# xieydd/crane-scheduler

Hardware: AMD Instinct MI355X
Metric: placements/sec (higher is better)
Workload: dtype f64

## Files before the change

crane-scheduler_amd/csrc/engine.hip:

```cpp
#include <hip/hip_runtime.h>

#include <algorithm>
#include <chrono>
#include <cmath>
#include <cstdio>
#include <cstdlib>
#include <cstring>
#include <memory>
#include <mutex>
#include <string>
#include <vector>

#include "../../include/crane_dyn.h"
#include "bindings.hpp"
#include "dyn_types.hpp"
#include "kernels.hpp"

using namespace crane;

namespace {

hipError_t before_free() { return crane::tl_aql ? crane::aql_wait(crane::tl_aql) : hipSuccess; }

template <typename T>
// ... 517 lines not shown
            HIPTRY(h, launch_step_one(s, st));
            h->reset_deferred = h->defer_reset;
            pk = k1.next;
            k1.on = false;
        } else if (pk.on && mine && pk.q == tl_aql) {
            HIPTRY(h, launch_k3s_delta_pods(h->N, h->node_offset, pk.P, pk.keys, pk.stt, pk.g, pk.perm, pk.pnow,
                                            pk.tiles, h->sd->bnode.p, h->N, d, adj.p, *pods, st));
            pk.on = false;
        } else {
            d.trace = h->trace_region(0);
            if ((pods ? pods->ntiles : 0) + (L + 1023) / 1024 > kTraceWgs) d.trace = nullptr;
            HIPTRY(h, launch_hot_count_delta(h->sd->bnode.p, h->N, d, adj.p, st, pods));
        }
        if (pods_done) *pods_done = pods != nullptr && pods->P > 0;
        h->delta_first = true;
        h->delta_chunks = (L + 1023) / 1024;
    }
    h->dl_adj_dirty[ab] = true;
    h->dl_pending = true;
    *done = true;
    return CRANE_OK;
}

static int hot_values_locked(crane_dyn* h, int64_t now_ns, int64_t hv_ts_ns, hipStream_t st,
                             const PodPrep* pods = nullptr, bool* pods_done = nullptr) {
    if (pods_done) *pods_done = false;
    h->delta_first = false;
    h->reset_deferred = false;
    if (h->N < 0) return h->fail(CRANE_E_STATE, "upload nodes before refreshing hot values");
    DevPolicy& dp = h->dp;
    HotCutoffs cut{};
// ... 1550 lines not shown
```

crane-scheduler_amd/csrc/hotcount.hip:

```cpp
#include <hip/hip_runtime.h>

#include <algorithm>

#include "dyn_types.hpp"
#include "kernels.hpp"
#include "pods.hpp"
#include "lds_hash.hpp"
#include "step_node.hpp"

namespace crane {

__device__ __forceinline__ int window_rank(int64_t ts, const HotCutoffs& cut) {
    int j = 0;
#pragma unroll
    for (int w = 0; w < kMaxWin; ++w)
        if (w < cut.n_win) j += ts > cut.sorted[w] ? 1 : 0;
    return j;
}

constexpr int kXChunk = kHxRegion;


template <int BT, bool POS>
__device__ __forceinline__ void k2d_body(const int32_t blk, const int32_t* __restrict__ bnode,
// ... 149 lines not shown
    for (int k = 1; k <= 4; ++k) CRANE_TSTAMP(d.trace, blockIdx.x, k);
}

hipError_t launch_hot_count_delta(const int32_t* bnode, int64_t N, const HotDelta& d, uint32_t* adj, hipStream_t st,
                                  const PodPrep* pods) {
    constexpr int BT = 512;
    if (d.n_rng < 0 || d.n_rng > kMaxWin || d.n_win < 1 || d.n_win > kDeltaMaxWin || N >= (1LL << 27))
        return hipErrorInvalidValue;
    const int64_t L = d.n_rng > 0 ? d.start[d.n_rng] : 0;
    const int64_t nb = (L + kDeltaChunk - 1) / kDeltaChunk;
    PodPrep pp{};
    if (pods && pods->P > 0) pp = *pods;
    const int64_t grid = pp.ntiles + nb;
    if (grid == 0) return hipSuccess;
    if (grid >= (1LL << 31)) return hipErrorInvalidValue;
    size_t lds = sizeof(uint32_t) * 2 * (size_t)kDeltaSlots + sizeof(uint16_t) * kDeltaMaxWin * kDeltaChunk;
    if (pp.ntiles > 0) lds = std::max(lds, kK3pLds);
    return klaunch(pp.ntiles > 0 ? "k2_delta+k3p_pods" : "k2_delta", k2_delta_pods<BT>, dim3((unsigned)grid), dim3(BT),
                   lds, st, bnode, N, d, adj, pp);
}

template <int BT, int REG, bool POS>
__global__ __launch_bounds__(BT) __attribute__((amdgpu_waves_per_eu(BT == 1024 ? 8 : 1)))
void k2l_partition(const int32_t* __restrict__ bnode,
                                                    const int64_t* __restrict__ bts, int64_t B, int64_t N,
                                                    HotCutoffs cut, HotPart g, uint32_t* __restrict__ CO,
                                                    uint32_t* __restrict__ region) {
    constexpr int kPer = REG / BT;
    constexpr int kSlots = 2 * REG;
    extern __shared__ __attribute__((aligned(16))) uint32_t sh[];
    __shared__ uint32_t part[BT];
// ... 230 lines not shown
```

crane-scheduler_amd/csrc/kernels.hpp:

```cpp
#pragma once
#include <hip/hip_ext.h>
#include <hip/hip_runtime.h>
#include <stdint.h>

#include "aql.hpp"
#include "dyn_types.hpp"

namespace crane {

enum { kShape4x6 = 0, kShape8x8 = 1, kShape16x16 = 2 };

struct KernelTimer {
    virtual ~KernelTimer() = default;
    virtual void next(const char* name, hipEvent_t* start, hipEvent_t* stop) = 0;
};
extern thread_local KernelTimer* tl_ktimer;

template <typename... KArgs, typename... Args>
inline hipError_t klaunch(const char* name, void (*kernel)(KArgs...), dim3 grid, dim3 block, size_t lds,
                          hipStream_t st, Args... args) {
    if (tl_aql) {
        static_assert((sizeof(KArgs) + ... + 0) + 16 * sizeof...(KArgs) <= kAqlMaxArgs, "kernel arguments too large");
        alignas(16) unsigned char buf[kAqlMaxArgs];
        size_t off = 0;
// ... 231 lines not shown
    StepTables st;
    StepGeometry g;
    const int32_t* perm;
    const int64_t* pnow;
    const int64_t* tile_mm;
    const K1Args* k1;
    const K1Step* ks;
    long long* reset_keys;
    int64_t reset_P;
    const int32_t* bnode;
    const HotDelta* d;
    uint32_t* adj;
    const PodPrep* pods;
};
bool step_one_has(int shape);
int64_t step_one_workgroups(int64_t nk3s, int64_t N_k1, int64_t ntiles, int64_t delta_len);
extern const int kStepOneWgPerCu;
hipError_t launch_step_one(const StepOne& s, hipStream_t st);
hipError_t launch_keys_reset(long long* keys, int64_t P, hipStream_t st);
hipError_t launch_step_pods(const int64_t* now, const uint8_t* flags, int64_t P, long long* keys, int64_t* batch,
                            int64_t* batch_next,
                            const StepGeometry& g, int32_t* perm, int64_t* pnow, int64_t* tile_mm, hipStream_t s);
hipError_t launch_step_nodes(int shape, const void* rec, int64_t N, double wsum, int32_t noprio,
                             const StepTables& st, const StepGeometry& g, const int64_t* tile_mm, hipStream_t s);
hipError_t launch_step_pairs(int shape, int64_t N, int64_t node_offset, int64_t P, long long* keys,
                             const StepTables& st, const StepGeometry& g, const int32_t* perm, const int64_t* pnow,
                             const int64_t* tile_mm, hipStream_t s);
struct K1Step {
    const int64_t* tile_mm;
    const int64_t* batch;
// ... 37 lines not shown
```

crane-scheduler_amd/csrc/lds_hash.hpp:

```cpp
#pragma once
#include <hip/hip_runtime.h>

#include <cstdint>

#include "kernels.hpp"

namespace crane {

constexpr int kDSlots = 4096;

template <int SLOTS = kDSlots>
__device__ __forceinline__ int32_t hash_add(int32_t* hkey, uint32_t* hcnt, uint32_t* hist, int bb, int32_t key,
                                            uint32_t add) {
    constexpr int kBits = __builtin_ctz(SLOTS);
    uint32_t h = ((uint32_t)key * 2654435761u) >> (32 - kBits);
    for (;;) {
        const int32_t old = atomicCAS(&hkey[h], -1, key);
        if (old == -1 || old == key) {
            atomicAdd(&hcnt[h], add);
            if (old == -1) {
                atomicAdd(&hist[(key >> 3) >> bb], 1u);
                return (int32_t)h;
            }
            return -1;
// ... 15 lines not shown
        const int lead = __ffsll((long long)am) - 1;
        const int32_t kl = __builtin_amdgcn_readlane(key[u], lead);
        const uint64_t m = __ballot(ok && key[u] == kl);
        const bool mine = lane == lead || (ok && key[u] != kl);
        const int32_t slot = mine ? hash_add<SLOTS>(hkey, hcnt, hist, bb, lane == lead ? kl : key[u],
                                                    lane == lead ? (uint32_t)__popcll(m) : 1u)
                                  : -1;
        const uint64_t nm = __ballot(slot >= 0);
        if (slot >= 0) useg[nw + __popcll(nm & ((1ull << lane) - 1ull))] = (uint16_t)slot;
        nw += __popcll(nm);
    }
    return nw;
}

constexpr int kDeltaChunk = 1024;
constexpr int kDeltaSlots = 4 * kDeltaChunk;

template <int BT>
__device__ __forceinline__ void k2_delta_body(const int32_t blk, const int32_t* __restrict__ bnode, int64_t N,
                                              const HotDelta& d, uint32_t* __restrict__ adj) {
    constexpr int kPer = kDeltaChunk / BT;
    constexpr int kKeys = kPer * kDeltaMaxWin;
    extern __shared__ __attribute__((aligned(16))) uint32_t sh[];
    __shared__ uint32_t hist[32];
    int32_t* hkey = reinterpret_cast<int32_t*>(sh);
    uint32_t* hcnt = sh + kDeltaSlots;
    uint16_t* uniq = reinterpret_cast<uint16_t*>(hcnt + kDSlots);
    const int64_t L = d.start[d.n_rng];
    int64_t pos[kPer];
    int32_t nd[kPer];
#pragma unroll
    for (int u = 0; u < kPer; ++u) {
        const int64_t t = (int64_t)blk * kDeltaChunk + u * BT + threadIdx.x;
        int k = 0;
        for (int r = 1; r < d.n_rng; ++r) k += t >= d.start[r] ? 1 : 0;
        pos[u] = d.lo[k] + (t - d.start[k]);
        nd[u] = bnode[t < L ? pos[u] : d.lo[0]];
        if (t >= L) nd[u] = -1;
    }
    for (int i = threadIdx.x; i < kDeltaSlots; i += BT) {
        hkey[i] = -1;
        hcnt[i] = 0;
    }
    if (threadIdx.x < 32) hist[threadIdx.x] = 0;
    __syncthreads();
    int32_t key[kKeys];
#pragma unroll
    for (int u = 0; u < kPer; ++u) {
        const bool ok = nd[u] >= 0 && (int64_t)nd[u] < N;
#pragma unroll
        for (int r = 0; r < kDeltaMaxWin; ++r) {
            const bool ia = pos[u] >= d.a[r], ip = pos[u] >= d.p[r];
            key[u * kDeltaMaxWin + r] = ok && r < d.n_win && ia != ip ? ((nd[u] * 8 + r) << 1) | (ia ? 1 : 0) : -1;
        }
    }
    uint16_t* useg = uniq + (threadIdx.x >> 6) * (kKeys * 64);
    const uint32_t nw = wave_aggregate<kDeltaSlots, kKeys>(key, hkey, hcnt, hist, 24, useg);
    __syncthreads();
    for (uint32_t i = threadIdx.x & 63; i < nw; i += 64) {
        const int s = useg[i];
        const int32_t k = hkey[s];
        const uint32_t c = hcnt[s];
        atomicAdd(&adj[(int64_t)((k >> 1) & 7) * N + (k >> 4)], (k & 1) ? 0u - c : c);
    }
}


}
```

crane-scheduler_amd/csrc/step.hip:

```cpp
#include <hip/hip_runtime.h>

#include <algorithm>

#include "dyn_types.hpp"
#include "kernels.hpp"
#include "pods.hpp"
#include "lds_hash.hpp"
#include "step_node.hpp"
#include "k1stream_body.hpp"

#ifndef K3S_BUCKETS
#define K3S_BUCKETS 1
#endif
#ifndef K3_KWARM
#define K3_KWARM 1
#endif

namespace crane {

constexpr int kPodTile = 1024;

__global__ __launch_bounds__(kPodTile) void k3p_pods(PodPrep pp) {
    extern __shared__ __attribute__((aligned(16))) unsigned char lds[];
    k3p_tile<kPodTile>(blockIdx.x, pp, lds);
// ... 20 lines not shown
    if (n < N && (o.slot0 >= 0 || o.slot1 >= 0)) step_emit<PD, PR>(r, n, tmin, tmax, wsum, noprio, o, st, blockIdx.x, S1Out{s1l, nullptr, false, 2 * kStepSeg, 0});
    __syncthreads();
    step_sort_publish<kStepSeg>(s1l, s1s, sh, st, blockIdx.x);
    if (st.rows) {
        int64_t pre;
        tile_prefetch(st, &pre);
        const PieceScr ps{reinterpret_cast<unsigned char*>(s1l) + 32 * kStepSeg,
                          ((int)sizeof(s1l) - 32 * kStepSeg) / PieceScr::bytes_per_piece & ~3};
        step_pieces<kStepSeg>(sh, st, blockIdx.x, ps);
        step_tile_rows<kStepSeg>(s1l, s1s, sh, st, blockIdx.x, &pre, ps);
    }
}

constexpr int kK3sWaves = 8;
constexpr int kK3sThreads = kK3sWaves * 64;
constexpr int kK3sPPL = 1024 / kK3sThreads;
constexpr int kK3sPods = kK3sThreads * kK3sPPL;
constexpr int kK3sBlkPerWg = 64;
constexpr int kK3sListBlk = 64;
constexpr int kSearchBucketBits = 8, kSearchBuckets = 1 << kSearchBucketBits;
constexpr int kK3sRecList = 512;
constexpr int kK3sPieceList = 512;
static_assert(kK3sMaxBlk <= kK3sThreads, "at least one lane per producer block");
static_assert(4 * kK3sListBlk <= 256, "list entries index the item map in 8 bits");
static_assert(kK3sPods == kPodTile, "a workgroup resolves one K3p tile");

__device__ __forceinline__ void team_count_le(const Step1* __restrict__ b0, const Step1* __restrict__ b1,
                                              const int32_t n[2], const int64_t tl[2], const int64_t th[2], int sub,
                                              int lpb, int lead, int32_t out[4]) {
    const uint64_t team = lpb == 64 ? ~0ull : ((1ull << lpb) - 1ull) << lead;
    int32_t lo[4] = {0, 0, 0, 0}, hi[4] = {n[0], n[0], n[1], n[1]};
    const int64_t t[4] = {tl[0], th[0], tl[1], th[1]};
    while ((lo[0] < hi[0]) | (lo[1] < hi[1]) | (lo[2] < hi[2]) | (lo[3] < hi[3])) {
        bool le[4];
#pragma unroll
        for (int q = 0; q < 4; ++q) {
            const int32_t span = hi[q] - lo[q];
            const int32_t p = lo[q] + (int32_t)((int64_t)span * (sub + 1) / (lpb + 1));
// ... 31 lines not shown
}

struct K3sLds {
    int64_t tt[kK3sPods];
    int32_t tree[2 * kK3sPods];
    int32_t umax[2];
    int32_t wpre[4 * kK3sListBlk + 1];
    int32_t wjl[2 * kK3sListBlk];
    int32_t wpl[2 * kK3sListBlk];
    uint8_t imap[kK3sRecList + kK3sPieceList];
#if K3S_BUCKETS
    int32_t sfirst[2][kSearchBuckets + 1];
#endif
};

__device__ __forceinline__ void k3s_body(const int64_t b, const StepTables& st, const int32_t* __restrict__ perm,
                                         const int64_t* __restrict__ pnow, const int64_t* __restrict__ tile_mm,
                                         int64_t P, int64_t node_offset, int32_t R, long long* __restrict__ keys,
                                         K3sLds& lds) {
    int64_t* const tt = lds.tt;
    int32_t* const tree = lds.tree;
    int32_t* const umax = lds.umax;
    int32_t* const wpre = lds.wpre;
    int32_t* const wjl = lds.wjl;
    int32_t* const wpl = lds.wpl;
    uint8_t* const imap = lds.imap;
#if K3S_BUCKETS
    int32_t(*const sfirst)[kSearchBuckets + 1] = lds.sfirst;
#endif
    CRANE_TSTAMP(st.trace, b, 0);
    const int32_t r = (int32_t)(b % R);
    const int64_t grp = b / R;
    const int lane = threadIdx.x & 63;
    const int64_t* ts = tile_mm + kTileStat * grp;
    int32_t xc = 0, stride = 1, k0 = 0, m = 0;
    if (R % 8 == 0) {
        const int32_t g = r & 7, S = R >> 3, s = r >> 3;
        const int32_t per = st.nblk >> 3, rem = st.nblk & 7;
        const int32_t nc = per + (g < rem ? 1 : 0);
        xc = g * per + min(g, rem) + s;
        stride = S;
        m = nc > s ? (nc - s + S - 1) / S : 0;
    } else {
        const int32_t per = (st.nblk + R - 1) / R;
        k0 = min(st.nblk, r * per);
        m = min(st.nblk, k0 + per) - k0;
    }
    int32_t lpb = 64;
    while (lpb > 1 && lpb * m > kK3sThreads) lpb >>= 1;
    const int32_t j = threadIdx.x / lpb, sub = threadIdx.x & (lpb - 1);
    const bool own = j < m;
    const int64_t ob = xc + (int64_t)stride * (k0 + j);
    const int lead = lane - sub;
    int4 c = make_int4(0, 0, 0, 0);
    int4 row = make_int4(-1, -1, 0, 0);
    int2 prow = make_int2(0, 0);
    if (own) {
        c = reinterpret_cast<const int4*>(st.cnt)[ob];
        if (st.rows) row = st.rows[grp * st.nblk + ob];
        if (st.prow) prow = st.prow[grp * st.nblk + ob];
    }
    bool live[kK3sPPL], ds[kK3sPPL];
    int32_t pod[kK3sPPL];
    int32_t praw[kK3sPPL];
    int64_t pn[kK3sPPL];
#pragma unroll
    for (int u = 0; u < kK3sPPL; ++u) {
        const int64_t slot = grp * kK3sPods + u * kK3sThreads + threadIdx.x;
        live[u] = slot < P;
        const int64_t sc = live[u] ? slot : 0;
        praw[u] = perm[sc];
        pn[u] = pnow[sc];
    }
#pragma unroll
    for (int u = 0; u < kK3sPPL; ++u) {
        tt[u * kK3sThreads + threadIdx.x] = live[u] ? pn[u] : INT64_MAX;
        const int32_t pr = live[u] ? praw[u] : 0;
        ds[u] = pr < 0;
        pod[u] = pr & 0x7FFFFFFF;
    }
    const int64_t tsv = ts[lane < kTileStat ? lane : 0];
    for (int i = threadIdx.x; i < 2 * kK3sPods; i += kK3sThreads) tree[i] = -1;
    if (threadIdx.x < 2) umax[threadIdx.x] = -1;
    auto stat = [&](int k) {
        const uint32_t lo32 = (uint32_t)__builtin_amdgcn_readlane((int)(uint32_t)tsv, k);
        const uint32_t hi32 = (uint32_t)__builtin_amdgcn_readlane((int)(uint32_t)((uint64_t)tsv >> 32), k);
        return (int64_t)(((uint64_t)hi32 << 32) | lo32);
    };
    const int64_t tlo[2] = {stat(0), stat(2)}, thi[2] = {stat(1), stat(3)};
    const int32_t cn = (int32_t)stat(4), cd = (int32_t)stat(5);
    const int32_t klo[2] = {0, cn}, khi[2] = {cn, cn + cd};
    const bool any[2] = {cn > 0, cd > 0};
#if K3S_BUCKETS
    int32_t sbs[2];
#pragma unroll
    for (int T = 0; T < 2; ++T) {
        const uint64_t span = klo[T] < khi[T] ? (uint64_t)(thi[T] - tlo[T]) : 0ull;
// ... 46 lines not shown
    if (lists && own && sub == 0) {
        wpre[2 * j + 0] = max(0, jj[1] - jj[0]);
        wpre[2 * j + 1] = max(0, jj[3] - jj[2]);
        wpre[2 * m + 2 * j + 0] = nm[0];
        wpre[2 * m + 2 * j + 1] = nm[1];
        wjl[2 * j] = jj[0];
        wjl[2 * j + 1] = jj[2];
        wpl[2 * j] = pl[0];
        wpl[2 * j + 1] = pl[1];
    }
    __syncthreads();
    CRANE_TSTAMP(st.trace, b, 1);
    const int32_t E = 4 * m;
    auto bucket_table = [&]() {
#if K3S_BUCKETS
        static_assert(kK3sThreads == 2 * kSearchBuckets, "a lane per (kind, bucket)");
        const int T = threadIdx.x / kSearchBuckets, k = threadIdx.x % kSearchBuckets;
        if (klo[T] < khi[T]) {
            sfirst[T][k] = slot_lower(tt, klo[T], khi[T], tlo[T] + ((int64_t)k << sbs[T]));
            if (k == 0) sfirst[T][kSearchBuckets] = khi[T];
        }
#endif
    };
    int32_t nrec = 0, total = 0;
    if (lists) {
        if (threadIdx.x < 64) {
            const int32_t v = lane < E ? wpre[lane] : 0;
            int32_t carry = (int32_t)wave_scan_add((uint32_t)v);
            if (lane < E) wpre[lane] = carry - v;
            carry = __builtin_amdgcn_readlane(carry, 63);
            for (int32_t e0 = 64; e0 < E; e0 += 64) {
                const int32_t e = e0 + lane;
                const int32_t x = e < E ? wpre[e] : 0;
                const int32_t inc = (int32_t)wave_scan_add((uint32_t)x) + carry;
                if (e < E) wpre[e] = inc - x;
// ... 2 lines not shown
            if (lane == 0) wpre[E] = carry;
        }
        bucket_table();
        __syncthreads();
        nrec = wpre[2 * m];
        total = wpre[E];
    } else if (K3S_BUCKETS) {
        bucket_table();
        __syncthreads();
    }
    const bool piece_list = lists && total - nrec <= kK3sPieceList;
    const bool rec_list = lists && nrec <= kK3sRecList;
    bool upd = false;
    const int32_t i0 = rec_list ? 0 : nrec, i1 = piece_list ? total : nrec;
    if (i1 > i0) {
        for (int32_t e = threadIdx.x; e < E; e += kK3sThreads) {
            const int32_t a = max(wpre[e], i0), z = min(wpre[e + 1], i1);
            for (int32_t i = a; i < z; ++i) imap[i - i0] = (uint8_t)e;
        }
        __syncthreads();
        constexpr int kU = (kK3sRecList + kK3sPieceList) / kK3sThreads;
        Step1 r1[kU];
        Mid pm[kU];
        int32_t ee[kU];
#pragma unroll
        for (int u = 0; u < kU; ++u) {
            const int32_t it = i0 + u * kK3sThreads + (int32_t)threadIdx.x;
            ee[u] = -1;
            if (it >= i1) continue;
            const int32_t e = imap[it - i0];
            ee[u] = e;
            const bool rec = e < 2 * m;
            const int32_t ej = rec ? e : e - 2 * m, jb = ej >> 1, T = ej & 1, idx = it - wpre[e];
            const int64_t obj = xc + (int64_t)stride * (k0 + jb);
            if (rec) r1[u] = (st.single + s1_at(st, T, obj))[wjl[2 * jb + T] + idx];
            else pm[u] = st.mid[(int64_t)T * st.mpad + obj * st.mstride + wpl[ej] + idx];
        }
#pragma unroll
        for (int u = 0; u < kU; ++u) {
            const int32_t e = ee[u];
            if (e < 0) continue;
            const bool rec = e < 2 * m;
            const int T = (rec ? e : e - 2 * m) & 1;
            if (rec) {
                const int32_t sp = find(T, r1[u].bp);
                if (r1[u].k0 >= 0) tree_max(tree, klo[T], sp, r1[u].k0);
                if (r1[u].k1 >= 0) tree_max(tree, sp, khi[T], r1[u].k1);
                upd = true;
            } else {
                const Mid& q = pm[u];
                if (q.s <= tlo[T] && q.e > thi[T]) um[T] = max(um[T], q.key);
                else if (q.s <= thi[T] && q.e > tlo[T]) {
                    tree_max(tree, find(T, q.s), find(T, q.e), q.key);
                    upd = true;
                }
            }
        }
    }
    if (own && !rec_list) {
#pragma unroll
        for (int T = 0; T < 2; ++T) {
            for (int32_t i = jj[2 * T] + sub; i < jj[2 * T + 1]; i += lpb) {
                const Step1 q = base[T][i];
                const int32_t sp = find(T, q.bp);
                if (q.k0 >= 0) tree_max(tree, klo[T], sp, q.k0);
                if (q.k1 >= 0) tree_max(tree, sp, khi[T], q.k1);
                upd = true;
            }
        }
// ... 21 lines not shown
                    }
                }
            }
        }
    }
    CRANE_TSTAMP(st.trace, b, 2);
#pragma unroll
    for (int T = 0; T < 2; ++T) {
        um[T] = wave_max(um[T]);
        if (lane == 0 && um[T] >= 0) atomicMax(&umax[T], um[T]);
    }
    const bool tree_used = __syncthreads_or(upd);
    CRANE_TSTAMP(st.trace, b, 3);
    constexpr int kLevels = 11;
    static_assert(kK3sPods == 1 << (kLevels - 1), "a segment tree over the tile's 1024 slots");
    int32_t anc[kK3sPPL][kLevels];
    if (tree_used) {
#pragma unroll
        for (int u = 0; u < kK3sPPL; ++u)
#pragma unroll
            for (int l = 0; l < kLevels; ++l) anc[u][l] = tree[(u * kK3sThreads + threadIdx.x + kK3sPods) >> l];
    }
#pragma unroll
    for (int u = 0; u < kK3sPPL; ++u) {
        int32_t best = umax[ds[u] ? 1 : 0];
        if (tree_used) {
#pragma unroll
            for (int l = 0; l < kLevels; ++l) best = max(best, anc[u][l]);
        }
        if (live[u] && best >= 0) {
            const int64_t sc = best >> 24;
            const int64_t n = 0xFFFFFF - (best & 0xFFFFFF);
            atomicMax(&keys[pod[u]],
                      (long long)((sc << 32) | (int64_t)(0xFFFFFFFFull - (uint64_t)(node_offset + n))));
        }
    }
    CRANE_TSTAMP(st.trace, b, 4);
}

int step_breakpoints(int shape) {
    switch (shape) {
        case kShape4x6: return 6 + 2;
        case kShape8x8: return 8 + 2;
        default: return 16 + 2;
    }
}

__global__ __launch_bounds__(kK3sThreads) void k3s_eval(StepTables st, const int32_t* __restrict__ perm,
                                                        const int64_t* __restrict__ pnow,
                                                        const int64_t* __restrict__ tile_mm, int64_t P,
                                                        int64_t node_offset, int32_t R,
                                                        long long* __restrict__ keys) {
#if K3_KWARM
    kernarg_warm<(int)sizeof(StepTables) + 64>();
#endif
    __shared__ K3sLds lds;
    k3s_body((int64_t)blockIdx.x, st, perm, pnow, tile_mm, P, node_offset, R, keys, lds);
}

struct K3sArgs {
    StepTables st;
    const int32_t* perm;
    const int64_t* pnow;
    const int64_t* tile_mm;
    int64_t P, node_offset;
    int32_t R;
    long long* keys;
};
static_assert(kK3sThreads == 512, "the fused launch's workgroups are the delta form's and K3p's 512 lanes");

__global__ __launch_bounds__(kK3sThreads) void k3s_delta_pods(K3sArgs k, int32_t nk3s, const int32_t* __restrict__ bnode,
                                                              int64_t N, HotDelta d, uint32_t* __restrict__ adj,
                                                              PodPrep pp) {
#if K3_KWARM
    kernarg_warm<(int)(sizeof(K3sArgs) + 32 + sizeof(HotDelta) + 8 + sizeof(PodPrep))>();
#endif
    const int64_t b = blockIdx.x;
    if (b < nk3s) {
        __shared__ K3sLds lds;
        k3s_body(b, k.st, k.perm, k.pnow, k.tile_mm, k.P, k.node_offset, k.R, k.keys, lds);
        return;
    }
    extern __shared__ __attribute__((aligned(16))) unsigned char dyn_lds[];
    if (b - nk3s < pp.ntiles) k3p_tile<kK3sThreads>(b - nk3s, pp, dyn_lds);
    else k2_delta_body<kK3sThreads>((int32_t)(b - nk3s - pp.ntiles), bnode, N, d, adj);
}

struct KeyReset {
    long long* keys;
    int64_t P;
};
constexpr size_t kDeltaLds = sizeof(uint32_t) * 2 * (size_t)kDeltaSlots + sizeof(uint16_t) * kDeltaMaxWin * kDeltaChunk;
constexpr size_t cmax(size_t a, size_t b) { return a > b ? a : b; }
constexpr size_t kStepOneLds = cmax(cmax(sizeof(K1Lds<4, 6>), sizeof(K3sLds)), cmax(kK3pLds, kDeltaLds));
static_assert(kStepOneLds >= sizeof(K1Lds<4, 6>) && kStepOneLds >= sizeof(K3sLds) && kStepOneLds >= kK3pLds &&
                  kStepOneLds >= kDeltaLds,
              "the union holds the largest body");
static_assert(kStepOneLds + 512 <= 53 * 1024, "three workgroups per compute unit (160 KiB)");
const int kStepOneWgPerCu = (int)std::min<size_t>(160 * 1024 / (kStepOneLds + 512), 4 * (K1S_WAVES - 1) / kK3sWaves);
constexpr int kOneK3sEnd = (int)sizeof(K3sArgs) + 16;
constexpr int kOneK1End = kOneK3sEnd + (int)sizeof(KeyReset) + (int)sizeof(K1Args) + (int)sizeof(K1Step) + 8;
constexpr int kOneEnd = kOneK1End + 16 + (int)sizeof(HotDelta) + 8 + (int)sizeof(PodPrep);

template <bool FULL>
__global__ __launch_bounds__(kK3sThreads) __attribute__((amdgpu_waves_per_eu(FULL ? K1S_WAVES : K1S_WAVES - 1)))
void step_one_launch(K3sArgs k, int32_t nk3s, int32_t nk1, int32_t nk1pad, KeyReset kr, K1Args a, K1Step step,
                     const int32_t* __restrict__ bnode, int64_t N, HotDelta d, uint32_t* __restrict__ adj, PodPrep pp) {
    extern __shared__ __attribute__((aligned(16))) unsigned char dyn_lds[];
    int64_t b = blockIdx.x;
    if (b < nk3s) {
#if K3_KWARM
        kernarg_warm<kOneK3sEnd>();
#endif
        k3s_body(b, k.st, k.perm, k.pnow, k.tile_mm, k.P, k.node_offset, k.R, k.keys,
                 *reinterpret_cast<K3sLds*>(dyn_lds));
        return;
    }
    b -= nk3s;
    if (b < nk1pad) {
        if (b >= nk1) return;
        if (threadIdx.x >= 256) {
            for (int64_t p = b * 256 + (threadIdx.x - 256); p < kr.P; p += (int64_t)nk1 * 256) kr.keys[p] = -1;
            return;
        }
        k1_stream_body<4, 6, FULL, kOneK1End>(a, step, b, nk1, *reinterpret_cast<K1Lds<4, 6>*>(dyn_lds));
        return;
    }
    b -= nk1pad;
#if K3_KWARM
    kernarg_warm<kOneEnd, kOneK1End>();
#endif
    if (b < pp.ntiles) k3p_tile<kK3sThreads>(b, pp, dyn_lds);
    else k2_delta_body<kK3sThreads>((int32_t)(b - pp.ntiles), bnode, N, d, adj);
}

__global__ __launch_bounds__(256) void keys_reset(long long* __restrict__ keys, int64_t P) {
    const int64_t p = (int64_t)blockIdx.x * 256 + threadIdx.x;
    if (p < P) keys[p] = -1;
}

StepGeometry step_geometry(int64_t P, int64_t N, int32_t nblk, int32_t blk_per_wg) {
    StepGeometry g{};
    g.nseg = (N + kStepSeg - 1) / kStepSeg;
    g.npad = g.nseg * kStepSeg;
    g.ntiles = (P + kPodTile - 1) / kPodTile;
    g.ngroups = (P + kK3sPods - 1) / kK3sPods;
    constexpr int64_t kMaxWg = 2048;
    const int32_t bpw = blk_per_wg > 0 ? blk_per_wg : kK3sBlkPerWg;
// ... 37 lines not shown
}

hipError_t launch_k3s_delta_pods(int64_t N_k3s, int64_t node_offset, int64_t P_k3s, long long* keys_k3s,
                                 const StepTables& st, const StepGeometry& g, const int32_t* perm, const int64_t* pnow,
                                 const int64_t* tile_mm, const int32_t* bnode, int64_t N, const HotDelta& d,
                                 uint32_t* adj, const PodPrep& pods, hipStream_t s) {
    if (P_k3s <= 0 || N_k3s <= 0 || d.n_win < 1 || d.n_win > kDeltaMaxWin || d.n_rng < 0 || d.n_rng > kMaxWin ||
        N >= (1LL << 27))
        return hipErrorInvalidValue;
    const int64_t nk = g.ngroups * g.R;
    const int64_t L = d.n_rng > 0 ? d.start[d.n_rng] : 0;
    const int64_t grid = nk + (pods.P > 0 ? pods.ntiles : 0) + (L + kDeltaChunk - 1) / kDeltaChunk;
    if (grid >= (1LL << 31) || nk >= (1LL << 31)) return hipErrorInvalidValue;
    PodPrep pp{};
    if (pods.P > 0) pp = pods;
    const size_t lds = std::max(kK3pLds, sizeof(uint32_t) * 2 * (size_t)kDeltaSlots +
                                             sizeof(uint16_t) * kDeltaMaxWin * kDeltaChunk);
    static const hipError_t attr = hipFuncSetAttribute((const void*)k3s_delta_pods,
                                                       hipFuncAttributeMaxDynamicSharedMemorySize, (int)lds);
    if (attr != hipSuccess) return attr;
    const K3sArgs k{st, perm, pnow, tile_mm, P_k3s, node_offset, g.R, keys_k3s};
    return klaunch("k3s_eval+k2_delta+k3p_pods", k3s_delta_pods, dim3((unsigned)grid), dim3(kK3sThreads), lds, s, k,
                   (int32_t)nk, bnode, N, d, adj, pp);
}

bool step_one_has(int shape) { return shape == kShape4x6; }

int64_t step_one_workgroups(int64_t nk3s, int64_t N_k1, int64_t ntiles, int64_t delta_len) {
    const int64_t nk1 = (N_k1 + 255) / 256;
    return nk3s + (nk1 + 7) / 8 * 8 + ntiles + (delta_len + kDeltaChunk - 1) / kDeltaChunk;
}

hipError_t launch_step_one(const StepOne& s, hipStream_t st) {
    const bool k3s = s.P_k3s > 0 && s.N > 0, k1 = s.k1 && s.ks && s.k1->N > 0;
    const bool delta = s.d != nullptr, pods = s.pods && s.pods->P > 0;
    if (delta && (s.d->n_win < 1 || s.d->n_win > kDeltaMaxWin || s.d->n_rng < 0 || s.d->n_rng > kMaxWin ||
                  s.N >= (1LL << 27)))
        return hipErrorInvalidValue;
    if (k1 && (s.k1->threads != 256 || s.k1->out || s.k1->hx_region || !s.ks->st.stage)) return hipErrorInvalidValue;
    const int64_t nk = k3s ? s.g.ngroups * s.g.R : 0;
    const int64_t nk1 = k1 ? (s.k1->N + 255) / 256 : 0, nk1pad = (nk1 + 7) / 8 * 8;
    const int64_t L = delta && s.d->n_rng > 0 ? s.d->start[s.d->n_rng] : 0;
    const int64_t grid = nk + nk1pad + (pods ? s.pods->ntiles : 0) + (L + kDeltaChunk - 1) / kDeltaChunk;
    if (grid >= (1LL << 31)) return hipErrorInvalidValue;
    if (grid == 0) return hipSuccess;
    const K3sArgs k{s.st, s.perm, s.pnow, s.tile_mm, k3s ? s.P_k3s : 0, s.node_offset, s.g.R, s.keys_k3s};
    const KeyReset kr{s.reset_keys, k1 && s.reset_keys ? s.reset_P : 0};
    const K1Args a = k1 ? *s.k1 : K1Args{};
    const K1Step ks = k1 ? *s.ks : K1Step{};
    const HotDelta d = delta ? *s.d : HotDelta{};
    const PodPrep pp = pods ? *s.pods : PodPrep{};
    const bool full = K1S_FULL && k1 && a.pol.npd == 4 && a.pol.npr == 6 && a.pol.n_win == kFullWin;
    static const hipError_t attr[2] = {
        hipFuncSetAttribute((const void*)step_one_launch<false>, hipFuncAttributeMaxDynamicSharedMemorySize,
                            (int)kStepOneLds),
        hipFuncSetAttribute((const void*)step_one_launch<true>, hipFuncAttributeMaxDynamicSharedMemorySize,
                            (int)kStepOneLds)};
    if (attr[full] != hipSuccess) return attr[full];
    const char* nm = "k3s_eval+k1_stream_steps+k2_delta+k3p_pods";
    return full ? klaunch(nm, step_one_launch<true>, dim3((unsigned)grid), dim3(kK3sThreads), kStepOneLds, st, k,
                          (int32_t)nk, (int32_t)nk1, (int32_t)nk1pad, kr, a, ks, s.bnode, s.N, d, s.adj, pp)
                : klaunch(nm, step_one_launch<false>, dim3((unsigned)grid), dim3(kK3sThreads), kStepOneLds, st, k,
                          (int32_t)nk, (int32_t)nk1, (int32_t)nk1pad, kr, a, ks, s.bnode, s.N, d, s.adj, pp);
}

hipError_t launch_keys_reset(long long* keys, int64_t P, hipStream_t st) {
    if (P <= 0 || !keys) return hipSuccess;
    return klaunch("keys_reset", keys_reset, dim3((unsigned)((P + 255) / 256)), dim3(256), 0, st, keys, P);
}

hipError_t launch_step_pairs(int shape, int64_t N, int64_t node_offset, int64_t P, long long* keys,
                             const StepTables& st, const StepGeometry& g, const int32_t* perm, const int64_t* pnow,
                             const int64_t* tile_mm, hipStream_t s) {
    (void)shape;
    if (P <= 0 || N <= 0) return hipSuccess;
    const dim3 grid((unsigned)(g.ngroups * g.R)), blk(kK3sThreads);
    return klaunch("k3s_eval", k3s_eval, grid, blk, 0, s, st, perm, pnow, tile_mm, P, node_offset, g.R, keys);
}
// ... 3 lines not shown
```

Baseline: 1.957 billion.

## Shrink fused step kernel to 256-thread workgroups and split key reset into own workgroups

Templates the k3s and delta bodies on thread count and launches the fused step_one kernel with 256 threads instead of 512. The delta chunk is halved and its LDS footprint resized, so more workgroups fit per compute unit. Key reset moves from the idle upper half of k1 workgroups into dedicated reset workgroups. The aim is higher occupancy and less wasted lanes in the mixed-role launch, at the cost of more per-lane serial work in k3s and a larger grid.

Result: faster. 2.334 billion (median of 6 runs) (+19.2%).

```diff
diff --git a/crane-scheduler_amd/csrc/engine.hip b/crane-scheduler_amd/csrc/engine.hip
--- a/crane-scheduler_amd/csrc/engine.hip
+++ b/crane-scheduler_amd/csrc/engine.hip
@@ -555,7 +555,7 @@
         }
         if (pods_done) *pods_done = pods != nullptr && pods->P > 0;
         h->delta_first = true;
-        h->delta_chunks = (L + 1023) / 1024;
+        h->delta_chunks = (L + kStepOneDeltaChunk - 1) / kStepOneDeltaChunk;
     }
     h->dl_adj_dirty[ab] = true;
     h->dl_pending = true;
diff --git a/crane-scheduler_amd/csrc/hotcount.hip b/crane-scheduler_amd/csrc/hotcount.hip
--- a/crane-scheduler_amd/csrc/hotcount.hip
+++ b/crane-scheduler_amd/csrc/hotcount.hip
@@ -187,7 +187,8 @@
     const int64_t grid = pp.ntiles + nb;
     if (grid == 0) return hipSuccess;
     if (grid >= (1LL << 31)) return hipErrorInvalidValue;
-    size_t lds = sizeof(uint32_t) * 2 * (size_t)kDeltaSlots + sizeof(uint16_t) * kDeltaMaxWin * kDeltaChunk;
+    size_t lds = delta_lds_bytes(kDeltaChunk, BT);
+    static_assert(delta_lds_bytes(kDeltaChunk, BT) <= 64 * 1024, "within a workgroup's LDS");
     if (pp.ntiles > 0) lds = std::max(lds, kK3pLds);
     return klaunch(pp.ntiles > 0 ? "k2_delta+k3p_pods" : "k2_delta", k2_delta_pods<BT>, dim3((unsigned)grid), dim3(BT),
                    lds, st, bnode, N, d, adj, pp);
diff --git a/crane-scheduler_amd/csrc/kernels.hpp b/crane-scheduler_amd/csrc/kernels.hpp
--- a/crane-scheduler_amd/csrc/kernels.hpp
+++ b/crane-scheduler_amd/csrc/kernels.hpp
@@ -269,6 +269,7 @@
     const PodPrep* pods;
 };
 bool step_one_has(int shape);
+constexpr int kStepOneDeltaChunk = 512;
 int64_t step_one_workgroups(int64_t nk3s, int64_t N_k1, int64_t ntiles, int64_t delta_len);
 extern const int kStepOneWgPerCu;
 hipError_t launch_step_one(const StepOne& s, hipStream_t st);
diff --git a/crane-scheduler_amd/csrc/lds_hash.hpp b/crane-scheduler_amd/csrc/lds_hash.hpp
--- a/crane-scheduler_amd/csrc/lds_hash.hpp
+++ b/crane-scheduler_amd/csrc/lds_hash.hpp
@@ -53,31 +53,41 @@
 }
 
 constexpr int kDeltaChunk = 1024;
-constexpr int kDeltaSlots = 4 * kDeltaChunk;
+constexpr int delta_slots(int chunk) { return 2 * kDeltaMaxWin * chunk; }
+constexpr size_t delta_lds_bytes(int chunk, int threads) {
+    return sizeof(uint32_t) * 2 * (size_t)delta_slots(chunk) +
+           sizeof(uint16_t) * (size_t)(threads / 64) * (size_t)(chunk / threads * kDeltaMaxWin * 64);
+}
 
-template <int BT>
+template <int BT, int CHUNK = kDeltaChunk>
 __device__ __forceinline__ void k2_delta_body(const int32_t blk, const int32_t* __restrict__ bnode, int64_t N,
                                               const HotDelta& d, uint32_t* __restrict__ adj) {
-    constexpr int kPer = kDeltaChunk / BT;
+    static_assert(CHUNK % BT == 0 && BT % 64 == 0, "whole bindings per lane, whole waves");
+    constexpr int kSlots = delta_slots(CHUNK);
+    static_assert((kSlots & (kSlots - 1)) == 0 && kSlots <= 65536, "hash_add masks the slot; uniq holds it in 16 bits");
+    constexpr int kPer = CHUNK / BT;
     constexpr int kKeys = kPer * kDeltaMaxWin;
+    static_assert(sizeof(uint32_t) * 2 * (size_t)kSlots + sizeof(uint16_t) * (BT / 64) * (kKeys * 64) ==
+                      delta_lds_bytes(CHUNK, BT),
+                  "the launchers' footprint is this layout's");
     extern __shared__ __attribute__((aligned(16))) uint32_t sh[];
     __shared__ uint32_t hist[32];
     int32_t* hkey = reinterpret_cast<int32_t*>(sh);
-    uint32_t* hcnt = sh + kDeltaSlots;
-    uint16_t* uniq = reinterpret_cast<uint16_t*>(hcnt + kDSlots);
+    uint32_t* hcnt = sh + kSlots;
+    uint16_t* uniq = reinterpret_cast<uint16_t*>(hcnt + kSlots);
     const int64_t L = d.start[d.n_rng];
     int64_t pos[kPer];
     int32_t nd[kPer];
 #pragma unroll
     for (int u = 0; u < kPer; ++u) {
-        const int64_t t = (int64_t)blk * kDeltaChunk + u * BT + threadIdx.x;
+        const int64_t t = (int64_t)blk * CHUNK + u * BT + threadIdx.x;
         int k = 0;
         for (int r = 1; r < d.n_rng; ++r) k += t >= d.start[r] ? 1 : 0;
         pos[u] = d.lo[k] + (t - d.start[k]);
         nd[u] = bnode[t < L ? pos[u] : d.lo[0]];
         if (t >= L) nd[u] = -1;
     }
-    for (int i = threadIdx.x; i < kDeltaSlots; i += BT) {
+    for (int i = threadIdx.x; i < kSlots; i += BT) {
         hkey[i] = -1;
         hcnt[i] = 0;
     }
@@ -94,7 +104,7 @@
         }
     }
     uint16_t* useg = uniq + (threadIdx.x >> 6) * (kKeys * 64);
-    const uint32_t nw = wave_aggregate<kDeltaSlots, kKeys>(key, hkey, hcnt, hist, 24, useg);
+    const uint32_t nw = wave_aggregate<kSlots, kKeys>(key, hkey, hcnt, hist, 24, useg);
     __syncthreads();
     for (uint32_t i = threadIdx.x & 63; i < nw; i += 64) {
         const int s = useg[i];
diff --git a/crane-scheduler_amd/csrc/step.hip b/crane-scheduler_amd/csrc/step.hip
--- a/crane-scheduler_amd/csrc/step.hip
+++ b/crane-scheduler_amd/csrc/step.hip
@@ -58,14 +58,12 @@
 
 constexpr int kK3sWaves = 8;
 constexpr int kK3sThreads = kK3sWaves * 64;
-constexpr int kK3sPPL = 1024 / kK3sThreads;
-constexpr int kK3sPods = kK3sThreads * kK3sPPL;
+constexpr int kK3sPods = 1024;
 constexpr int kK3sBlkPerWg = 64;
 constexpr int kK3sListBlk = 64;
 constexpr int kSearchBucketBits = 8, kSearchBuckets = 1 << kSearchBucketBits;
 constexpr int kK3sRecList = 512;
 constexpr int kK3sPieceList = 512;
-static_assert(kK3sMaxBlk <= kK3sThreads, "at least one lane per producer block");
 static_assert(4 * kK3sListBlk <= 256, "list entries index the item map in 8 bits");
 static_assert(kK3sPods == kPodTile, "a workgroup resolves one K3p tile");
 
@@ -127,6 +125,7 @@
 #endif
 };
 
+template <int TH>
 __device__ __forceinline__ void k3s_body(const int64_t b, const StepTables& st, const int32_t* __restrict__ perm,
                                          const int64_t* __restrict__ pnow, const int64_t* __restrict__ tile_mm,
                                          int64_t P, int64_t node_offset, int32_t R, long long* __restrict__ keys,
@@ -138,6 +137,8 @@
     int32_t* const wjl = lds.wjl;
     int32_t* const wpl = lds.wpl;
     uint8_t* const imap = lds.imap;
+    static_assert(kK3sPods % TH == 0 && TH % 64 == 0 && kK3sMaxBlk <= TH, "whole pods per lane, a lane per producer block");
+    constexpr int kPPL = kK3sPods / TH;
 #if K3S_BUCKETS
     int32_t(*const sfirst)[kSearchBuckets + 1] = lds.sfirst;
 #endif
@@ -160,7 +161,7 @@
         m = min(st.nblk, k0 + per) - k0;
     }
     int32_t lpb = 64;
-    while (lpb > 1 && lpb * m > kK3sThreads) lpb >>= 1;
+    while (lpb > 1 && lpb * m > TH) lpb >>= 1;
     const int32_t j = threadIdx.x / lpb, sub = threadIdx.x & (lpb - 1);
     const bool own = j < m;
     const int64_t ob = xc + (int64_t)stride * (k0 + j);
@@ -173,27 +174,23 @@
         if (st.rows) row = st.rows[grp * st.nblk + ob];
         if (st.prow) prow = st.prow[grp * st.nblk + ob];
     }
-    bool live[kK3sPPL], ds[kK3sPPL];
-    int32_t pod[kK3sPPL];
-    int32_t praw[kK3sPPL];
-    int64_t pn[kK3sPPL];
-#pragma unroll
-    for (int u = 0; u < kK3sPPL; ++u) {
-        const int64_t slot = grp * kK3sPods + u * kK3sThreads + threadIdx.x;
-        live[u] = slot < P;
-        const int64_t sc = live[u] ? slot : 0;
+    int32_t praw[kPPL];
+    int64_t pn[kPPL];
+#pragma unroll
+    for (int u = 0; u < kPPL; ++u) {
+        const int64_t slot = grp * kK3sPods + u * TH + threadIdx.x;
+        const int64_t sc = slot < P ? slot : 0;
         praw[u] = perm[sc];
         pn[u] = pnow[sc];
     }
 #pragma unroll
-    for (int u = 0; u < kK3sPPL; ++u) {
-        tt[u * kK3sThreads + threadIdx.x] = live[u] ? pn[u] : INT64_MAX;
-        const int32_t pr = live[u] ? praw[u] : 0;
-        ds[u] = pr < 0;
-        pod[u] = pr & 0x7FFFFFFF;
+    for (int u = 0; u < kPPL; ++u) {
+        const bool live = grp * kK3sPods + u * TH + threadIdx.x < P;
+        tt[u * TH + threadIdx.x] = live ? pn[u] : INT64_MAX;
+        if (!live) praw[u] = 0;
     }
     const int64_t tsv = ts[lane < kTileStat ? lane : 0];
-    for (int i = threadIdx.x; i < 2 * kK3sPods; i += kK3sThreads) tree[i] = -1;
+    for (int i = threadIdx.x; i < 2 * kK3sPods; i += TH) tree[i] = -1;
     if (threadIdx.x < 2) umax[threadIdx.x] = -1;
     auto stat = [&](int k) {
         const uint32_t lo32 = (uint32_t)__builtin_amdgcn_readlane((int)(uint32_t)tsv, k);
@@ -270,11 +267,14 @@
     const int32_t E = 4 * m;
     auto bucket_table = [&]() {
 #if K3S_BUCKETS
-        static_assert(kK3sThreads == 2 * kSearchBuckets, "a lane per (kind, bucket)");
-        const int T = threadIdx.x / kSearchBuckets, k = threadIdx.x % kSearchBuckets;
-        if (klo[T] < khi[T]) {
-            sfirst[T][k] = slot_lower(tt, klo[T], khi[T], tlo[T] + ((int64_t)k << sbs[T]));
-            if (k == 0) sfirst[T][kSearchBuckets] = khi[T];
+        static_assert(2 * kSearchBuckets % TH == 0, "whole rounds over (kind, bucket)");
+#pragma unroll
+        for (int q = threadIdx.x; q < 2 * kSearchBuckets; q += TH) {
+            const int T = q / kSearchBuckets, k = q % kSearchBuckets;
+            if (klo[T] < khi[T]) {
+                sfirst[T][k] = slot_lower(tt, klo[T], khi[T], tlo[T] + ((int64_t)k << sbs[T]));
+                if (k == 0) sfirst[T][kSearchBuckets] = khi[T];
+            }
         }
 #endif
     };
@@ -307,45 +307,49 @@
     bool upd = false;
     const int32_t i0 = rec_list ? 0 : nrec, i1 = piece_list ? total : nrec;
     if (i1 > i0) {
-        for (int32_t e = threadIdx.x; e < E; e += kK3sThreads) {
+        for (int32_t e = threadIdx.x; e < E; e += TH) {
             const int32_t a = max(wpre[e], i0), z = min(wpre[e + 1], i1);
             for (int32_t i = a; i < z; ++i) imap[i - i0] = (uint8_t)e;
         }
         __syncthreads();
-        constexpr int kU = (kK3sRecList + kK3sPieceList) / kK3sThreads;
-        Step1 r1[kU];
-        Mid pm[kU];
-        int32_t ee[kU];
-#pragma unroll
-        for (int u = 0; u < kU; ++u) {
-            const int32_t it = i0 + u * kK3sThreads + (int32_t)threadIdx.x;
-            ee[u] = -1;
-            if (it >= i1) continue;
-            const int32_t e = imap[it - i0];
-            ee[u] = e;
-            const bool rec = e < 2 * m;
-            const int32_t ej = rec ? e : e - 2 * m, jb = ej >> 1, T = ej & 1, idx = it - wpre[e];
-            const int64_t obj = xc + (int64_t)stride * (k0 + jb);
-            if (rec) r1[u] = (st.single + s1_at(st, T, obj))[wjl[2 * jb + T] + idx];
-            else pm[u] = st.mid[(int64_t)T * st.mpad + obj * st.mstride + wpl[ej] + idx];
-        }
-#pragma unroll
-        for (int u = 0; u < kU; ++u) {
-            const int32_t e = ee[u];
-            if (e < 0) continue;
-            const bool rec = e < 2 * m;
-            const int T = (rec ? e : e - 2 * m) & 1;
-            if (rec) {
-                const int32_t sp = find(T, r1[u].bp);
-                if (r1[u].k0 >= 0) tree_max(tree, klo[T], sp, r1[u].k0);
-                if (r1[u].k1 >= 0) tree_max(tree, sp, khi[T], r1[u].k1);
-                upd = true;
-            } else {
-                const Mid& q = pm[u];
-                if (q.s <= tlo[T] && q.e > thi[T]) um[T] = max(um[T], q.key);
-                else if (q.s <= thi[T] && q.e > tlo[T]) {
-                    tree_max(tree, find(T, q.s), find(T, q.e), q.key);
+        constexpr int kU = 2, kPass = (kK3sRecList + kK3sPieceList) / (kU * TH);
+#pragma unroll
+        for (int h = 0; h < kPass; ++h) {
+            if (i0 + h * kU * TH >= i1) break;
+            Step1 r1[kU];
+            Mid pm[kU];
+            int32_t ee[kU];
+#pragma unroll
+            for (int u = 0; u < kU; ++u) {
+                const int32_t it = i0 + (h * kU + u) * TH + (int32_t)threadIdx.x;
+                ee[u] = -1;
+                if (it >= i1) continue;
+                const int32_t e = imap[it - i0];
+                ee[u] = e;
+                const bool rec = e < 2 * m;
+                const int32_t ej = rec ? e : e - 2 * m, jb = ej >> 1, T = ej & 1, idx = it - wpre[e];
+                const int64_t obj = xc + (int64_t)stride * (k0 + jb);
+                if (rec) r1[u] = (st.single + s1_at(st, T, obj))[wjl[2 * jb + T] + idx];
+                else pm[u] = st.mid[(int64_t)T * st.mpad + obj * st.mstride + wpl[ej] + idx];
+            }
+#pragma unroll
+            for (int u = 0; u < kU; ++u) {
+                const int32_t e = ee[u];
+                if (e < 0) continue;
+                const bool rec = e < 2 * m;
+                const int T = (rec ? e : e - 2 * m) & 1;
+                if (rec) {
+                    const int32_t sp = find(T, r1[u].bp);
+                    if (r1[u].k0 >= 0) tree_max(tree, klo[T], sp, r1[u].k0);
+                    if (r1[u].k1 >= 0) tree_max(tree, sp, khi[T], r1[u].k1);
                     upd = true;
+                } else {
+                    const Mid& q = pm[u];
+                    if (q.s <= tlo[T] && q.e > thi[T]) um[T] = max(um[T], q.key);
+                    else if (q.s <= thi[T] && q.e > tlo[T]) {
+                        tree_max(tree, find(T, q.s), find(T, q.e), q.key);
+                        upd = true;
+                    }
                 }
             }
         }
@@ -397,26 +401,35 @@
     CRANE_TSTAMP(st.trace, b, 3);
     constexpr int kLevels = 11;
     static_assert(kK3sPods == 1 << (kLevels - 1), "a segment tree over the tile's 1024 slots");
-    int32_t anc[kK3sPPL][kLevels];
-    if (tree_used) {
-#pragma unroll
-        for (int u = 0; u < kK3sPPL; ++u)
-#pragma unroll
-            for (int l = 0; l < kLevels; ++l) anc[u][l] = tree[(u * kK3sThreads + threadIdx.x + kK3sPods) >> l];
-    }
-#pragma unroll
-    for (int u = 0; u < kK3sPPL; ++u) {
-        int32_t best = umax[ds[u] ? 1 : 0];
+    constexpr int kV = 2;
+    static_assert(kPPL % kV == 0, "whole passes");
+#pragma unroll
+    for (int h = 0; h < kPPL / kV; ++h) {
+        int32_t anc[kV][kLevels];
         if (tree_used) {
 #pragma unroll
-            for (int l = 0; l < kLevels; ++l) best = max(best, anc[u][l]);
-        }
-        if (live[u] && best >= 0) {
-            const int64_t sc = best >> 24;
-            const int64_t n = 0xFFFFFF - (best & 0xFFFFFF);
-            atomicMax(&keys[pod[u]],
-                      (long long)((sc << 32) | (int64_t)(0xFFFFFFFFull - (uint64_t)(node_offset + n))));
-        }
+            for (int v = 0; v < kV; ++v)
+#pragma unroll
+                for (int l = 0; l < kLevels; ++l)
+                    anc[v][l] = tree[((h * kV + v) * TH + threadIdx.x + kK3sPods) >> l];
+        }
+#pragma unroll
+        for (int v = 0; v < kV; ++v) {
+            const int u = h * kV + v;
+            int32_t best = umax[praw[u] < 0 ? 1 : 0];
+            if (tree_used) {
+#pragma unroll
+                for (int l = 0; l < kLevels; ++l) best = max(best, anc[v][l]);
+            }
+            const bool live = grp * kK3sPods + u * TH + threadIdx.x < P;
+            if (live && best >= 0) {
+                const int64_t sc = best >> 24;
+                const int64_t n = 0xFFFFFF - (best & 0xFFFFFF);
+                atomicMax(&keys[praw[u] & 0x7FFFFFFF],
+                          (long long)((sc << 32) | (int64_t)(0xFFFFFFFFull - (uint64_t)(node_offset + n))));
+            }
+        }
+        if (h + 1 < kPPL / kV) asm volatile("" ::: "memory");
     }
     CRANE_TSTAMP(st.trace, b, 4);
 }
@@ -438,7 +451,7 @@
     kernarg_warm<(int)sizeof(StepTables) + 64>();
 #endif
     __shared__ K3sLds lds;
-    k3s_body((int64_t)blockIdx.x, st, perm, pnow, tile_mm, P, node_offset, R, keys, lds);
+    k3s_body<kK3sThreads>((int64_t)blockIdx.x, st, perm, pnow, tile_mm, P, node_offset, R, keys, lds);
 }
 
 struct K3sArgs {
@@ -461,7 +474,7 @@
     const int64_t b = blockIdx.x;
     if (b < nk3s) {
         __shared__ K3sLds lds;
-        k3s_body(b, k.st, k.perm, k.pnow, k.tile_mm, k.P, k.node_offset, k.R, k.keys, lds);
+        k3s_body<kK3sThreads>(b, k.st, k.perm, k.pnow, k.tile_mm, k.P, k.node_offset, k.R, k.keys, lds);
         return;
     }
     extern __shared__ __attribute__((aligned(16))) unsigned char dyn_lds[];
@@ -473,48 +486,59 @@
     long long* keys;
     int64_t P;
 };
-constexpr size_t kDeltaLds = sizeof(uint32_t) * 2 * (size_t)kDeltaSlots + sizeof(uint16_t) * kDeltaMaxWin * kDeltaChunk;
+constexpr int kStepOneThreads = 256;
+constexpr int kResetPerWg = 4 * kStepOneThreads;
+static_assert(kResetPerWg == kPodTile, "step_one_workgroups counts a reset workgroup per pod tile");
+constexpr size_t kStepOneDeltaLds = delta_lds_bytes(kStepOneDeltaChunk, kStepOneThreads);
 constexpr size_t cmax(size_t a, size_t b) { return a > b ? a : b; }
-constexpr size_t kStepOneLds = cmax(cmax(sizeof(K1Lds<4, 6>), sizeof(K3sLds)), cmax(kK3pLds, kDeltaLds));
+constexpr size_t kStepOneLds = cmax(cmax(sizeof(K1Lds<4, 6>), sizeof(K3sLds)), cmax(kK3pLds, kStepOneDeltaLds));
 static_assert(kStepOneLds >= sizeof(K1Lds<4, 6>) && kStepOneLds >= sizeof(K3sLds) && kStepOneLds >= kK3pLds &&
-                  kStepOneLds >= kDeltaLds,
+                  kStepOneLds >= kStepOneDeltaLds,
               "the union holds the largest body");
-static_assert(kStepOneLds + 512 <= 53 * 1024, "three workgroups per compute unit (160 KiB)");
-const int kStepOneWgPerCu = (int)std::min<size_t>(160 * 1024 / (kStepOneLds + 512), 4 * (K1S_WAVES - 1) / kK3sWaves);
+static_assert(kStepOneLds == sizeof(K3sLds), "no body asks for more than K3s");
+static_assert(7 * (kStepOneLds + 512) <= 160 * 1024, "seven workgroups per compute unit (160 KiB)");
+const int kStepOneWgPerCu =
+    (int)std::min<size_t>(160 * 1024 / (kStepOneLds + 512), 4 * (K1S_WAVES - 1) / (kStepOneThreads / 64));
 constexpr int kOneK3sEnd = (int)sizeof(K3sArgs) + 16;
 constexpr int kOneK1End = kOneK3sEnd + (int)sizeof(KeyReset) + (int)sizeof(K1Args) + (int)sizeof(K1Step) + 8;
 constexpr int kOneEnd = kOneK1End + 16 + (int)sizeof(HotDelta) + 8 + (int)sizeof(PodPrep);
 
 template <bool FULL>
-__global__ __launch_bounds__(kK3sThreads) __attribute__((amdgpu_waves_per_eu(FULL ? K1S_WAVES : K1S_WAVES - 1)))
-void step_one_launch(K3sArgs k, int32_t nk3s, int32_t nk1, int32_t nk1pad, KeyReset kr, K1Args a, K1Step step,
-                     const int32_t* __restrict__ bnode, int64_t N, HotDelta d, uint32_t* __restrict__ adj, PodPrep pp) {
+__global__ __launch_bounds__(kStepOneThreads) __attribute__((amdgpu_waves_per_eu(FULL ? K1S_WAVES : K1S_WAVES - 1)))
+void step_one_launch(K3sArgs k, int32_t nk3s, int32_t nk1, int32_t nk1pad, int32_t nreset, KeyReset kr, K1Args a,
+                     K1Step step, const int32_t* __restrict__ bnode, int64_t N, HotDelta d, uint32_t* __restrict__ adj,
+                     PodPrep pp) {
     extern __shared__ __attribute__((aligned(16))) unsigned char dyn_lds[];
     int64_t b = blockIdx.x;
     if (b < nk3s) {
 #if K3_KWARM
         kernarg_warm<kOneK3sEnd>();
 #endif
-        k3s_body(b, k.st, k.perm, k.pnow, k.tile_mm, k.P, k.node_offset, k.R, k.keys,
-                 *reinterpret_cast<K3sLds*>(dyn_lds));
+        k3s_body<kStepOneThreads>(b, k.st, k.perm, k.pnow, k.tile_mm, k.P, k.node_offset, k.R, k.keys,
+                                  *reinterpret_cast<K3sLds*>(dyn_lds));
         return;
     }
     b -= nk3s;
     if (b < nk1pad) {
         if (b >= nk1) return;
-        if (threadIdx.x >= 256) {
-            for (int64_t p = b * 256 + (threadIdx.x - 256); p < kr.P; p += (int64_t)nk1 * 256) kr.keys[p] = -1;
-            return;
-        }
         k1_stream_body<4, 6, FULL, kOneK1End>(a, step, b, nk1, *reinterpret_cast<K1Lds<4, 6>*>(dyn_lds));
         return;
     }
     b -= nk1pad;
+    if (b < nreset) {
+#pragma unroll
+        for (int u = 0; u < kResetPerWg / kStepOneThreads; ++u) {
+            const int64_t p = b * kResetPerWg + u * kStepOneThreads + threadIdx.x;
+            if (p < kr.P) kr.keys[p] = -1;
+        }
+        return;
+    }
+    b -= nreset;
 #if K3_KWARM
     kernarg_warm<kOneEnd, kOneK1End>();
 #endif
-    if (b < pp.ntiles) k3p_tile<kK3sThreads>(b, pp, dyn_lds);
-    else k2_delta_body<kK3sThreads>((int32_t)(b - pp.ntiles), bnode, N, d, adj);
+    if (b < pp.ntiles) k3p_tile<kStepOneThreads>(b, pp, dyn_lds);
+    else k2_delta_body<kStepOneThreads, kStepOneDeltaChunk>((int32_t)(b - pp.ntiles), bnode, N, d, adj);
 }
 
 __global__ __launch_bounds__(256) void keys_reset(long long* __restrict__ keys, int64_t P) {
@@ -582,8 +606,8 @@
     if (grid >= (1LL << 31) || nk >= (1LL << 31)) return hipErrorInvalidValue;
     PodPrep pp{};
     if (pods.P > 0) pp = pods;
-    const size_t lds = std::max(kK3pLds, sizeof(uint32_t) * 2 * (size_t)kDeltaSlots +
-                                             sizeof(uint16_t) * kDeltaMaxWin * kDeltaChunk);
+    constexpr size_t lds = cmax(kK3pLds, delta_lds_bytes(kDeltaChunk, kK3sThreads));
+    static_assert(lds + sizeof(K3sLds) <= 64 * 1024, "beside K3s's static LDS in a workgroup's 64 KiB");
     static const hipError_t attr = hipFuncSetAttribute((const void*)k3s_delta_pods,
                                                        hipFuncAttributeMaxDynamicSharedMemorySize, (int)lds);
     if (attr != hipSuccess) return attr;
@@ -596,7 +620,7 @@
 
 int64_t step_one_workgroups(int64_t nk3s, int64_t N_k1, int64_t ntiles, int64_t delta_len) {
     const int64_t nk1 = (N_k1 + 255) / 256;
-    return nk3s + (nk1 + 7) / 8 * 8 + ntiles + (delta_len + kDeltaChunk - 1) / kDeltaChunk;
+    return nk3s + (nk1 + 7) / 8 * 8 + 2 * ntiles + (delta_len + kStepOneDeltaChunk - 1) / kStepOneDeltaChunk;
 }
 
 hipError_t launch_step_one(const StepOne& s, hipStream_t st) {
@@ -609,11 +633,13 @@
     const int64_t nk = k3s ? s.g.ngroups * s.g.R : 0;
     const int64_t nk1 = k1 ? (s.k1->N + 255) / 256 : 0, nk1pad = (nk1 + 7) / 8 * 8;
     const int64_t L = delta && s.d->n_rng > 0 ? s.d->start[s.d->n_rng] : 0;
-    const int64_t grid = nk + nk1pad + (pods ? s.pods->ntiles : 0) + (L + kDeltaChunk - 1) / kDeltaChunk;
+    const KeyReset kr{s.reset_keys, k1 && s.reset_keys && s.reset_P > 0 ? s.reset_P : 0};
+    const int64_t nreset = (kr.P + kResetPerWg - 1) / kResetPerWg;
+    const int64_t grid = nk + nk1pad + nreset + (pods ? s.pods->ntiles : 0) +
+                         (L + kStepOneDeltaChunk - 1) / kStepOneDeltaChunk;
     if (grid >= (1LL << 31)) return hipErrorInvalidValue;
     if (grid == 0) return hipSuccess;
     const K3sArgs k{s.st, s.perm, s.pnow, s.tile_mm, k3s ? s.P_k3s : 0, s.node_offset, s.g.R, s.keys_k3s};
-    const KeyReset kr{s.reset_keys, k1 && s.reset_keys ? s.reset_P : 0};
     const K1Args a = k1 ? *s.k1 : K1Args{};
     const K1Step ks = k1 ? *s.ks : K1Step{};
     const HotDelta d = delta ? *s.d : HotDelta{};
@@ -626,10 +652,10 @@
                             (int)kStepOneLds)};
     if (attr[full] != hipSuccess) return attr[full];
     const char* nm = "k3s_eval+k1_stream_steps+k2_delta+k3p_pods";
-    return full ? klaunch(nm, step_one_launch<true>, dim3((unsigned)grid), dim3(kK3sThreads), kStepOneLds, st, k,
-                          (int32_t)nk, (int32_t)nk1, (int32_t)nk1pad, kr, a, ks, s.bnode, s.N, d, s.adj, pp)
-                : klaunch(nm, step_one_launch<false>, dim3((unsigned)grid), dim3(kK3sThreads), kStepOneLds, st, k,
-                          (int32_t)nk, (int32_t)nk1, (int32_t)nk1pad, kr, a, ks, s.bnode, s.N, d, s.adj, pp);
+    return full ? klaunch(nm, step_one_launch<true>, dim3((unsigned)grid), dim3(kStepOneThreads), kStepOneLds, st, k,
+                          (int32_t)nk, (int32_t)nk1, (int32_t)nk1pad, (int32_t)nreset, kr, a, ks, s.bnode, s.N, d, s.adj, pp)
+                : klaunch(nm, step_one_launch<false>, dim3((unsigned)grid), dim3(kStepOneThreads), kStepOneLds, st, k,
+                          (int32_t)nk, (int32_t)nk1, (int32_t)nk1pad, (int32_t)nreset, kr, a, ks, s.bnode, s.N, d, s.adj, pp);
 }
 
 hipError_t launch_keys_reset(long long* keys, int64_t P, hipStream_t st) {
```
